# matthewdm0816/BridgeQA

Hardware: AMD Instinct MI355X
Metric: train samples/s (40k-pt scene + 512^2 view, bs16) (higher is better)
Workload: dtype bf16

## Files before the change

bridgeqa_amd/_ext.py:

```python
import ctypes
import os

import torch

from . import _cabi, gemm_route
from .gemm_route import GEMM_TILE_ROWS, TILE256_MIN_K, pick_tile

_LIB_PATH = os.environ.get("BQHIP_LIB") or os.path.join(os.path.dirname(os.path.abspath(__file__)), "lib", "libbqhip.so")

if not os.path.exists(_LIB_PATH):
    raise ImportError(
        "bridgeqa_amd: %s is missing -- build it with `python -m bridgeqa_amd.build` "
        "(hipcc --offload-arch=gfx950). There is no CPU fallback." % _LIB_PATH)

_lib = ctypes.CDLL(_LIB_PATH)
_D = _cabi.DEFINES
_cabi.bind(_lib, ("bq_abi_version", "bq_last_error"))
ABI_VERSION = _D["BQHIP_ABI_VERSION"]
if _lib.bq_abi_version() != ABI_VERSION:
    raise ImportError("bridgeqa_amd: libbqhip.so ABI %d != %d (stale library: python -m bridgeqa_amd.build --force)"
                      % (_lib.bq_abi_version(), ABI_VERSION))
_cabi.bind(_lib)
_cabi.bind(_lib, _cabi.ADDITIVE_PROTOS)
_cabi.bind(_lib, _cabi.EXTENSION_PROTOS)
# ... 1120 lines not shown
            raise RuntimeError("%s must be a contiguous float32 tensor" % n)
    W, H = int(image_dims[0]), int(image_dims[1])
    F, N = depth.shape[0], points.shape[0]
    if depth.numel() != F * W * H or frames.shape != (F, 40) or points.shape[1] != 3:
        raise RuntimeError("project_points: shapes %s %s %s" % (tuple(points.shape), tuple(depth.shape), tuple(frames.shape)))
    with torch.cuda.device(points.device):
        pix = torch.empty(F, N, dtype=torch.int32, device=points.device)
        _check(_lib.bq_project_points(_p(points), _p(depth), _p(frames), _p(pix), F, N, W, H, float(fx), float(fy), float(cx),
                                      float(cy), float(depth_min), float(depth_max), float(accuracy), _stream()),
               "project_points")
    return pix


def fuse_point_features(pix, feat, maxpool):
    if not (pix.is_cuda and feat.is_cuda):
        raise RuntimeError("fuse_point_features: CPU not supported")
    if pix.dtype != torch.int32 or feat.dtype != torch.float32 or not pix.is_contiguous() or not feat.is_contiguous():
        raise RuntimeError("fuse_point_features: pix must be contiguous int32, feat contiguous float32")
    F, N = pix.shape
    if feat.dim() != 3 or feat.shape[0] != F:
        raise RuntimeError("fuse_point_features: feat must be (F, H*W, C)")
    HW, C = feat.shape[1], feat.shape[2]
    with torch.cuda.device(pix.device):
        out = torch.empty(N, C, dtype=torch.float32, device=pix.device)
        _check(_lib.bq_fuse_point_features(_p(pix), _p(feat), _p(out), F, N, HW, C, int(bool(maxpool)), _stream()),
               "fuse_point_features")
    return out


GEMM_P_XC, GEMM_Q_XC, GEMM_OUT_F32, GEMM_BACKGROUND = (_D["BQ_GEMM_" + n] for n in ("P_XC", "Q_XC", "OUT_F32", "BACKGROUND"))
EPI_NONE, EPI_BIAS, EPI_BIAS_GELU, EPI_DGELU, EPI_BIAS_CE, EPI_ADD = (
    _D["BQ_GEMM_EPI_" + n] for n in ("NONE", "BIAS", "BIAS_GELU", "DGELU", "BIAS_CE", "ADD"))
GEMM_DET = _D["BQ_GEMM_DET"]
_GemmDesc = _cabi.STRUCTS["bq_gemm_desc"]


def _mat(t, name):
    if not t.is_cuda:
        raise RuntimeError("%s: CPU not supported (bridgeqa_amd has no CPU path)" % name)
    if t.dim() != 2 or t.stride(1) != 1:
        raise RuntimeError("%s must be a 2-D tensor with a contiguous last dimension" % name)
    return t


def _mat_rows(t, name):
    if not t.is_cuda:
        raise RuntimeError("%s: CPU not supported (bridgeqa_amd has no CPU path)" % name)
    if t.dim() == 2:
        if t.stride(1) != 1:
            raise RuntimeError("%s must have a contiguous last dimension" % name)
        return (t.shape[0], t.shape[1]), t.stride(0), 0, 0
    if t.dim() != 3 or t.stride(2) != 1:
        raise RuntimeError("%s must be (rows, cols) or a (batch, rows, cols) view with a contiguous last dimension" % name)
    B, R, C = t.shape
    ld, bs = t.stride(1), t.stride(0)
    if B == 1 or bs == R * ld:
        return (B * R, C), ld, 0, 0
    if bs < R * ld or bs % 8 or R > 65535:
        raise RuntimeError("%s: unsupported batched-row view (stride %s, shape %s)" % (name, t.stride(), tuple(t.shape)))
    return (B * R, C), ld, R, bs


def gemm_grouped(problems, flags, epilogue=EPI_NONE, tile=None, fixed_order=False):
    if _det() or fixed_order:
        return _gemm_grouped_det(problems, flags, epilogue, tile)
    return _gemm_grouped_launch(problems, flags, epilogue, tile)
# ... 6 lines not shown
    oshape, ldo, o_rpb, o_bs = _mat_rows(out, "out")
    if P.dtype != torch.bfloat16 or Q.dtype != torch.bfloat16:
        raise RuntimeError("gemm: operands must be bf16")
    if out.dtype != (torch.float32 if f32 else torch.bfloat16):
        raise RuntimeError("gemm: out must be %s" % ("float32" if f32 else "bfloat16"))
    Ni, Kc = (P.shape[1], P.shape[0]) if pxc else (P.shape[0], P.shape[1])
    Nj, Kq = (qshape[1], qshape[0]) if qxc else (qshape[0], qshape[1])
    Ni = int(pr.get("Ni", Ni))
    if (Kq != Kc and "Kc" not in pr) or tuple(oshape) != (Nj, Ni):
        raise RuntimeError("gemm: shape mismatch P%s Q%s out%s" % (tuple(P.shape), tuple(Q.shape), tuple(out.shape)))
    d.P, d.Q, d.out = P.data_ptr(), Q.data_ptr(), out.data_ptr()
    bias, out2, aux, colsum = pr.get("bias"), pr.get("out2"), pr.get("aux"), pr.get("colsum")
    if bias is not None and (bias.dtype not in (torch.float32, torch.bfloat16) or bias.numel() != Ni
                             or not bias.is_contiguous()):
        raise RuntimeError("gemm: bias must be a contiguous fp32 or bf16 (Ni,) tensor")
    d.bias_bf16 = int(bias is not None and bias.dtype == torch.bfloat16)
    n_cs = Nj if (pxc and qxc and f32) else Ni
    if epilogue != EPI_BIAS_CE and colsum is not None and (colsum.dtype != torch.float32 or colsum.numel() != n_cs
                                                           or not colsum.is_contiguous()):
        raise RuntimeError("gemm: colsum must be a contiguous fp32 (%d,) tensor" % n_cs)
    for t, nm in ((out2, "out2"), (aux, "aux")):
        if epilogue != EPI_BIAS_CE and t is not None and (t.dtype != torch.bfloat16 or t.shape != out.shape
                                                          or t.stride() != out.stride()):
            raise RuntimeError("gemm: %s must be bf16 and laid out like out" % nm)
    d.bias, d.out2, d.aux, d.colsum = _p(bias), _p(out2), _p(aux), _p(colsum)
    d.ldp, d.ldq, d.ldo = P.stride(0), ldq, ldo
    d.q_rpb, d.q_bstride, d.o_rpb, d.o_bstride = q_rpb, q_bs, o_rpb, o_bs
    d.accum = int(bool(pr.get("accum", False)))
    d.Ni, d.Nj, d.Kc = Ni, Nj, int(pr.get("Kc", Kc))
    d.p_bytes, d.q_bytes, d.ksplit = int(pr.get("p_bytes", 0)), int(pr.get("q_bytes", 0)), int(pr.get("ksplit", 1))
    return gemm_route.Shape(Ni, Nj, d.Kc, colsum is not None, bool(q_rpb or o_rpb))


def _gemm_grouped_launch(problems, flags, epilogue, tile):
    n = len(problems)
    arr = (_GemmDesc * n)()
    shapes = [_gemm_pack(arr[k], pr, flags, epilogue) for k, pr in enumerate(problems)]
    tile = int(tile or gemm_route.auto_tile(shapes, flags, epilogue))
    dev = problems[0]["out"].device
    if tile != 128:
        flags &= ~GEMM_BACKGROUND
    with torch.cuda.device(dev):
        if tile == 128 and n == 1 and (STREAMK[0] or STREAMK256[0]):
            _streamk_workspace(dev)
        _check(_lib.bq_gemm_bf16(arr, n, int(flags), int(epilogue), tile, _stream()), "gemm_bf16")


def _gemm_grouped_det(problems, flags, epilogue, tile):
    if _det() and (STREAMK[0] or STREAMK256[0]):
        raise RuntimeError("gemm: stream-K is on (streamk_enable / streamk256_enable) while the deterministic mode is on")
    f32 = bool(flags & GEMM_OUT_F32)
    probs, folds, sums = [], [], []
    for pr in problems:
        ks = int(pr.get("ksplit", 1))
        if epilogue != EPI_BIAS_CE and ks > 1:
            out = pr["out"]
            if not f32 or pr.get("colsum") is not None or pr.get("accum") or out.dim() != 2 or out.stride(1) != 1:
                raise RuntimeError("gemm: a cut contraction in the deterministic mode needs fp32 plain-row out, no colsum or accum")
            slab = torch.empty(ks, out.shape[0], out.stride(0), dtype=torch.float32, device=out.device)
            folds.append((slab, out, ks))
            pr = dict(pr, out=slab[0, :, :out.shape[1]])
        elif not f32 and epilogue != EPI_BIAS_CE and pr.get("colsum") is not None:
            sums.append((pr["out"], pr["colsum"]))
            pr = dict(pr, colsum=None)
        probs.append(pr)
    _gemm_grouped_launch(probs, flags | GEMM_DET, epilogue, tile)
    for slab, out, ks in folds:
        R, C = out.shape
        with torch.cuda.device(out.device):
            _check(_det_entry("gemm_splitk_fold")(_p(slab), _p(out), None, ks, R, C, out.stride(0), _stream()),
# ... 499 lines not shown
```

bridgeqa_amd/csrc/gemm.hip:

```cpp
#include "gemm_common.h"

namespace bq {

typedef unsigned u32x4_sk __attribute__((ext_vector_type(4)));

template <bool P_XC, bool Q_XC, int EPI, bool OUT_F32, bool SK = false>
__global__ __launch_bounds__(512) void gemm256_kernel(const GemmArgs args) {
  static_assert(!SK || (!P_XC && !Q_XC && !OUT_F32 && (EPI == EPI_NONE || EPI == EPI_BIAS)), "stream-K: K-contiguous operands, bf16 out");
  __shared__ __attribute__((aligned(16))) unsigned char smem[131072];
  __shared__ unsigned s_skflag;
  constexpr bool GTAB = !OUT_F32 && (EPI == EPI_BIAS_GELU || EPI == EPI_DGELU);
  __shared__ float s_gtab[GTAB ? GELU_TAB_N : 1];
  const int tid = threadIdx.x;
  const int lane = tid & 63;
  const int wave = __builtin_amdgcn_readfirstlane(tid >> 6);
  const int wr = wave >> 2, wc = wave & 3;

  const int nwg = args.total_tiles;
  auto xcd_order = [](int b, int n) {
    const int q = n >> 3, r = n & 7, x = b & 7;
    return (x < r ? x * (q + 1) : r * (q + 1) + (x - r) * q) + (b >> 3);
  };
  const int G = (int)gridDim.x;
  const int nkt_full = SK ? (args.p[0].Kc + 63) >> 6 : 1;
  const int U = SK ? nwg * nkt_full : 0;
  auto bound = [&](int x) {
    int b = (int)((long)x * U / G);
    const int r = b % nkt_full;
    return r == 1 ? b - 1 : (r == nkt_full - 1 ? b + 1 : b);
  };
  const int slot = SK ? xcd_order((int)blockIdx.x, G) : 0;
  int su = SK ? bound(slot) : 0;
  const int sue = SK ? bound(slot + 1) : 0;
  if (SK && su >= sue) return;
  for (;;) {
  int t, kb = 0, kseg = 0;
  if (SK) {
    t = su / nkt_full;
    kb = su - t * nkt_full;
    kseg = min(nkt_full - kb, sue - su);
  } else {
    t = xcd_order((int)blockIdx.x, nwg);
  }
  int pi = 0;
  for (int k = 1; k < args.n; ++k)
    if (t >= args.p[k].tile0) pi = k;
  const GemmProblem &pr = args.p[pi];
  const int tl = t - pr.tile0;
  const int tiles_j = (pr.Nj + 255) >> 8;
  const int bj = tiles_j - 1 - tl / pr.tiles_i(), bi = tl % pr.tiles_i();
  const int i0 = bi * 256, j0 = bj * 256;
  const int Ni = pr.Ni, Nj = pr.Nj, Kc = pr.Kc;
  const int ldp = pr.ldp, ldq = pr.ldq;
  const int nkt = SK ? kseg : (Kc + 63) >> 6;

  const auto rsP = __builtin_amdgcn_make_buffer_rsrc((void *)pr.P, 0, pr.p_bytes, 0x00020000);
  const auto rsQ = __builtin_amdgcn_make_buffer_rsrc((void *)pr.Q, 0, pr.q_bytes, 0x00020000);
  const int ur = wave * 8 + (lane >> 3);
  const int cp = lane & 7;
  unsigned voff[8];
#pragma unroll
  for (int u = 0; u < 4; ++u) {
    const int g = u & 1, half = u >> 1;
    if (!P_XC) {
      const int c = cp ^ (ur & 7);
      voff[u] = (unsigned)(((i0 + g * 128 + half * 64 + ur) * ldp + c * 8) * 2);
    } else {
      const int c = cp ^ (xg(ur) << 1);
      voff[u] = (unsigned)((ur * ldp + i0 + g * 128 + half * 64 + c * 8) * 2);
    }
  }
#pragma unroll
  for (int u = 0; u < 4; ++u) {
    const int h = u & 1, half = u >> 1;
    if (!Q_XC) {
      const int c = cp ^ (ur & 7);
      voff[4 + u] = (unsigned)(((j0 + h * 128 + (ur >> 5) * 64 + half * 32 + (ur & 31)) * ldq + c * 8) * 2);
    } else {
      const int c = cp ^ (xg(ur) << 1);
      voff[4 + u] = (unsigned)((ur * ldq + j0 + h * 128 + (c >> 2) * 64 + half * 32 + (c & 3) * 8) * 2);
    }
  }
  const unsigned p_step = P_XC ? (unsigned)(64 * ldp * 2) : 128u;
  const unsigned q_step = Q_XC ? (unsigned)(64 * ldq * 2) : 128u;
  if (SK) {
#pragma unroll
    for (int u = 0; u < 4; ++u) { voff[u] += (unsigned)kb * p_step; voff[4 + u] += (unsigned)kb * q_step; }
  }
  const unsigned lds_w = (unsigned)(wave * 1024);
  const int q_rpb = Q_XC ? (int)pr.q_rpb() : 0;
  const unsigned q_gap = (unsigned)((pr.q_bstride - q_rpb * ldq) * 2);
  int q_rl[2] = {ur, ur};

  auto stage_pair = [&](int u, int kt) {
    const bool live = kt < nkt;
    const unsigned base = (unsigned)((kt & 1) * 65536 + u * 8192) + lds_w;
#pragma unroll
    for (int d = 0; d < 2; ++d) {
      const unsigned vo = live ? voff[u + d] : 0x80000000u;
      __builtin_amdgcn_raw_ptr_buffer_load_lds(u < 4 ? rsP : rsQ, (lds_void_t *)(smem + base + d * 8192), 16, vo, 0, 0, 0);
      voff[u + d] += (u < 4) ? p_step : q_step;
    }
    if (Q_XC && u >= 4 && q_rpb != 0) {
      int &rl = q_rl[(u - 4) >> 1];
      rl += 64;
      const bool wrap = rl >= q_rpb;
      rl -= wrap ? q_rpb : 0;
      voff[u] += wrap ? q_gap : 0u;
      voff[u + 1] += wrap ? q_gap : 0u;
    }
  };

  const int row16 = lane & 15, q4 = lane >> 4;
  const int kc_base = row16 * 128 + ((q4 ^ (row16 & 7)) << 4);
  int xc_base[4];
  {
    const int q = (lane & 15) >> 2, p = lane & 3, g = (q >> 1) | ((q4 & 1) << 1);
#pragma unroll
    for (int s = 0; s < 4; ++s) xc_base[s] = (8 * q4 + q) * 128 + ((s ^ g) << 5) + 8 * p;
  }
  const int uA0 = wr * 8192, uA1 = (2 + wr) * 8192, uB0 = (4 + (wc >> 1)) * 8192, uB1 = (6 + (wc >> 1)) * 8192;
  const int bsub = (wc & 1) * 2;

  const int iw = i0 + wr * 128, jw = j0 + wc * 64;
  const bool vA0 = iw < Ni, vA1 = iw + 64 < Ni, vB0 = jw < Nj, vB1 = jw + 32 < Nj;

  f32x4 acc[8][4];
#pragma unroll
  for (int a = 0; a < 8; ++a)
#pragma unroll
    for (int b = 0; b < 4; ++b) acc[a][b] = f32x4{0.f, 0.f, 0.f, 0.f};

  constexpr bool QSUM = P_XC && Q_XC && OUT_F32;
  const bool do_qsum = QSUM && pr.colsum != nullptr && bi == 0 && wr == 0;
  f32x4 qs[4];
  bf16x8 ones;
#pragma unroll
  for (int b = 0; b < 4; ++b) qs[b] = f32x4{0.f, 0.f, 0.f, 0.f};
#pragma unroll
  for (int e = 0; e < 8; ++e) ones[e] = (__bf16)1.0f;
#define BQ_MFMA_QSUM(FB, BO)                                                                          \
  if (QSUM && do_qsum) {                                                                              \
    _Pragma("unroll") for (int kk = 0; kk < 2; ++kk) _Pragma("unroll") for (int b = 0; b < 2; ++b)    \
        qs[BO + b] = __builtin_amdgcn_mfma_f32_16x16x32_bf16(ones, FB[b][kk], qs[BO + b], 0, 0, 0);   \
  }

  stage_pair(0, 0); stage_pair(4, 0); stage_pair(6, 0); stage_pair(2, 0); stage_pair(0, 1); stage_pair(4, 1); stage_pair(6, 1);
  if (GTAB) gelu_tab_fill<EPI == EPI_DGELU>(s_gtab, tid, 512);
  asm volatile("s_waitcnt vmcnt(8)" ::: "memory");
  BQ_BARRIER();
  if (wr == 1) BQ_BARRIER();

  bf16x8 fa[4][2], fb0[2][2], fb1[2][2];
  const unsigned smem_lds = lds_addr_of(smem);
#define BQ_MFMA_Q(AO, FB, BO)                                                                         \
  _Pragma("unroll") for (int kk = 0; kk < 2; ++kk) _Pragma("unroll") for (int a = 0; a < 4; ++a)      \
      _Pragma("unroll") for (int b = 0; b < 2; ++b) acc[AO + a][BO + b] =                             \
          __builtin_amdgcn_mfma_f32_16x16x32_bf16(fa[a][kk], FB[b][kk], acc[AO + a][BO + b], 0, 0, 0);
#define BQ_PHASE_SYNC_A()                                   \
  asm volatile("s_waitcnt vmcnt(8)" ::: "memory");          \
  asm volatile("s_waitcnt lgkmcnt(0)" ::: "memory");        \
  BQ_BARRIER();                                             \
  __builtin_amdgcn_sched_barrier(0);                        \
  __builtin_amdgcn_s_setprio(1);
#define BQ_PHASE_SYNC_B()                                   \
  __builtin_amdgcn_s_setprio(0);                            \
  BQ_BARRIER();

  for (int kt = 0; kt < nkt; ++kt) {
    const unsigned buf = smem_lds + (unsigned)((kt & 1) * 65536);
    if (vA0) {
#pragma unroll
      for (int a = 0; a < 4; ++a)
#pragma unroll
        for (int kk = 0; kk < 2; ++kk) fa[a][kk] = read_frag_asm<P_XC>(buf + uA0, a, kk, kc_base, xc_base);
    }
    if (vB0) {
#pragma unroll
      for (int b = 0; b < 2; ++b)
#pragma unroll
        for (int kk = 0; kk < 2; ++kk) fb0[b][kk] = read_frag_asm<Q_XC>(buf + uB0, bsub + b, kk, kc_base, xc_base);
    }
    if (vB1) {
#pragma unroll
      for (int b = 0; b < 2; ++b)
#pragma unroll
        for (int kk = 0; kk < 2; ++kk) fb1[b][kk] = read_frag_asm<Q_XC>(buf + uB1, bsub + b, kk, kc_base, xc_base);
    }
    stage_pair(2, kt + 1);
    BQ_PHASE_SYNC_A();
    if (vA0 && vB0) { BQ_MFMA_Q(0, fb0, 0) }
    if (vB0) { BQ_MFMA_QSUM(fb0, 0) }
    if (vA0 && vB1) { BQ_MFMA_Q(0, fb1, 2) }
    if (vB1) { BQ_MFMA_QSUM(fb1, 2) }
    BQ_PHASE_SYNC_B();
    if (vA1) {
#pragma unroll
      for (int a = 0; a < 4; ++a)
#pragma unroll
        for (int kk = 0; kk < 2; ++kk) fa[a][kk] = read_frag_asm<P_XC>(buf + uA1, a, kk, kc_base, xc_base);
    }
    stage_pair(0, kt + 2); stage_pair(4, kt + 2); stage_pair(6, kt + 2);
    BQ_PHASE_SYNC_A();
// ... 927 lines not shown
  for (int k = 0; k < ga.n; ++k) long_k = long_k && ga.p[k].Kc >= 64 * long_k_tiles;
  int rc = -1;
  with_gemm_form(pxc, qxc, f32, epi, [&](auto PX, auto QX, auto F32, auto E) {
    constexpr bool P = decltype(PX)::value, Q = decltype(QX)::value, F = decltype(F32)::value;
    constexpr int EP = decltype(E)::value;
    rc = det ? launch_variant<P, Q, EP, F, FORM_DET>(ga, tile, st, false) : launch_variant<P, Q, EP, F>(ga, tile, st, long_k);
  });
  return rc;
}

}

extern "C" int bq_gemm_max_problems(void) { return bq::GEMM_MAX_PROBLEMS; }

extern "C" int bq_gemm_bf16(const bq_gemm_desc *d, int n, int flags, int epilogue, int tile, void *stream) {
  using namespace bq;
  BQ_REQUIRE(epilogue >= BQ_GEMM_EPI_NONE && epilogue <= BQ_GEMM_EPI_ADD, BQ_EINVAL, "bq_gemm_bf16: unknown epilogue %d", epilogue);
  BQ_REQUIRE(d != nullptr && n >= 1, BQ_EINVAL, "bq_gemm_bf16: no problems");
  BQ_REQUIRE(tile == 256 || tile == 128 || tile == 64 || tile == 32, BQ_EINVAL,
             "bq_gemm_bf16: tile must be 256, 128 (= 256 x 128), 64 or 32 (got %d)", tile);
  const bool pxc = flags & BQ_GEMM_P_XC, qxc = flags & BQ_GEMM_Q_XC, f32 = flags & BQ_GEMM_OUT_F32;
  BQ_REQUIRE(!(flags & BQ_GEMM_BACKGROUND) || tile == 128, BQ_EINVAL, "bq_gemm_bf16: BQ_GEMM_BACKGROUND needs tile 128");
  const bool det = flags & BQ_GEMM_DET;
  BQ_REQUIRE(!det || tile != 128 || gemm_sk_mode() == 0, BQ_EINVAL,
             "bq_gemm_bf16: BQ_GEMM_DET with a stream-K mode on (bq_gemm_streamk_mode)");
  hipStream_t st = (hipStream_t)stream;
  int done = 0;
  while (done < n) {
    GemmArgs ga;
    ga.n = 0;
    ga.total_tiles = 0;
    while (done < n && ga.n < GEMM_MAX_PROBLEMS) {
      const bq_gemm_desc &s = d[done];
      BQ_REQUIRE(s.P && s.Q && s.out, BQ_EINVAL, "bq_gemm_bf16: null operand (problem %d)", done);
      BQ_REQUIRE(s.Ni > 0 && s.Nj > 0 && s.Kc > 0, BQ_EINVAL, "bq_gemm_bf16: empty problem %d", done);
      BQ_REQUIRE(s.ldp % 8 == 0 && s.ldq % 8 == 0, BQ_EINVAL, "bq_gemm_bf16: operand leading dimensions must be multiples of 8 elements");
      BQ_REQUIRE(s.Ni % 8 == 0 && s.ldo % (f32 ? 4 : 8) == 0, BQ_EINVAL, "bq_gemm_bf16: Ni and ldo must be multiples of 8 (Ni = %d, ldo = %d)", s.Ni, s.ldo);
      BQ_REQUIRE(!qxc || s.Nj % 8 == 0, BQ_EINVAL, "bq_gemm_bf16: a contraction-major Q needs Nj %% 8 == 0 (Nj = %d)", s.Nj);
      BQ_REQUIRE((pxc && qxc) || s.Kc % 64 == 0, BQ_EINVAL,
                 "bq_gemm_bf16: a K-contiguous operand needs Kc %% 64 == 0 (Kc = %d; zero-pad the other operand and pass "
                 "p_bytes / q_bytes when the rows are shorter)", s.Kc);
      BQ_REQUIRE(((uintptr_t)s.P % 16 == 0) && ((uintptr_t)s.Q % 16 == 0) && ((uintptr_t)s.out % 16 == 0), BQ_EINVAL,
                 "bq_gemm_bf16: operands must be 16-byte aligned");
      BQ_REQUIRE(epilogue != EPI_BIAS_GELU || s.out2, BQ_EINVAL, "bq_gemm_bf16: BIAS_GELU needs out2");
      BQ_REQUIRE(epilogue != EPI_DGELU || s.aux, BQ_EINVAL, "bq_gemm_bf16: DGELU needs aux");
      BQ_REQUIRE(epilogue != EPI_ADD || s.aux, BQ_EINVAL, "bq_gemm_bf16: ADD needs aux");
      BQ_REQUIRE((epilogue != EPI_ADD && epilogue != EPI_DGELU && tile != 128) || ((long)s.Nj + 256) * s.ldo * (f32 ? 4 : 2) < 0x7FFFFFFFL,
                 BQ_EINVAL, "bq_gemm_bf16: out / aux larger than 2 GB (problem %d)", done);
      const long pb = pxc ? ((long)(s.Kc - 1) * s.ldp + s.Ni) * 2 : ((long)(s.Ni - 1) * s.ldp + s.Kc) * 2;
      long qb = qxc ? ((long)(s.Kc - 1) * s.ldq + s.Nj) * 2 : ((long)(s.Nj - 1) * s.ldq + s.Kc) * 2;
      const int tj = tile == 256 ? 256 : tile, ti = (tile == 256 || tile == 128) ? 256 : 64;
      BQ_REQUIRE(s.q_rpb >= 0 && s.o_rpb >= 0 && s.q_rpb <= 65535 && s.o_rpb <= 65535, BQ_EINVAL,
                 "bq_gemm_bf16: q_rpb / o_rpb must be in 0..65535 (problem %d)", done);
      long q_span = 0, o_span = 0;
      if (s.q_rpb > 0) {
        const long rows = qxc ? s.Kc : s.Nj, cols = qxc ? s.Nj : s.Kc;
        BQ_REQUIRE(rows % s.q_rpb == 0 && s.q_bstride % 8 == 0 && (long)s.q_bstride >= (long)s.q_rpb * s.ldq, BQ_EINVAL,
                   "bq_gemm_bf16: q map: rows %ld must be whole batches of q_rpb = %d rows, q_bstride %% 8 == 0 and >= q_rpb * ldq",
                   rows, s.q_rpb);
        BQ_REQUIRE(tile != 256 || (qxc && s.q_rpb >= 64), BQ_EINVAL,
                   "bq_gemm_bf16: tile 256 maps only the contraction rows of a contraction-major Q, q_rpb >= 64");
        BQ_REQUIRE(tile != 128 || !qxc, BQ_EINVAL, "bq_gemm_bf16: tile 128 has no map on a contraction-major Q");
        q_span = (rows / s.q_rpb - 1) * (long)s.q_bstride + (long)(s.q_rpb - 1) * s.ldq + cols;
        qb = q_span * 2;
      }
      if (s.o_rpb > 0) {
// ... 9 lines not shown
      BQ_REQUIRE(pb + (long)ti * s.ldp * 2 < 0x7FFFFFFFL && qb + (long)tj * s.ldq * 2 + (s.q_rpb > 0 ? 2L * s.q_bstride * 2 : 0) < 0x7FFFFFFFL,
                 BQ_EINVAL, "bq_gemm_bf16: operand larger than 2 GB (problem %d)", done);
      BQ_REQUIRE(!det || f32 || epilogue == EPI_BIAS_CE || !s.colsum, BQ_EINVAL,
                 "bq_gemm_bf16: BQ_GEMM_DET: column sums of a bf16 output are float atomics (use bq_colsum_grouped_det_bf16)");
      BQ_REQUIRE(!det || epilogue == EPI_BIAS_CE || s.ksplit <= 1 || (!s.colsum && !s.accum && s.o_rpb == 0), BQ_EINVAL,
                 "bq_gemm_bf16: BQ_GEMM_DET: a cut contraction takes no colsum, accum or output map (problem %d)", done);
      GemmProblem &g = ga.p[ga.n];
      g.P = (const __bf16 *)s.P; g.Q = (const __bf16 *)s.Q; g.out = s.out; g.bias = s.bias; g.out2 = s.out2;
      g.aux = (const __bf16 *)s.aux; g.colsum = s.colsum;
      g.ldp = s.ldp; g.ldq = s.ldq; g.ldo = s.ldo; g.Ni = s.Ni; g.Nj = s.Nj; g.Kc = s.Kc;
      g.flags = (s.bias_bf16 != 0 ? 1 : 0) | (s.accum != 0 ? 2 : 0);
      g.rpb_pack = (int)((unsigned)s.q_rpb | ((unsigned)s.o_rpb << 16));
      g.q_bstride = s.q_bstride; g.o_bstride = s.o_bstride;
      g.p_bytes = (unsigned)(s.p_bytes > 0 ? s.p_bytes : pb);
      g.q_bytes = (unsigned)((s.q_bytes > 0 && s.q_rpb == 0) ? s.q_bytes : qb);
      int ks_ = 1;
      if (epilogue == EPI_BIAS_CE) {
        BQ_REQUIRE(s.out2 && s.aux && s.colsum && s.ksplit > 0 && s.ksplit <= s.Ni && s.ksplit <= 65535 && tile == 256, BQ_EINVAL,
                   "bq_gemm_bf16: the cross-entropy epilogue needs out2 (partials), aux (targets), colsum (target logits), "
                   "ksplit = valid vocabulary entries (<= 65535), tile 256");
        ks_ = s.ksplit;
      } else {
        BQ_REQUIRE(s.ksplit <= 1 || (f32 && tile != 256), BQ_EINVAL, "bq_gemm_bf16: ksplit needs fp32 out and tile 64");
        BQ_REQUIRE(s.ksplit <= 65535, BQ_ELIMIT, "bq_gemm_bf16: ksplit = %d > 65535", s.ksplit);
        BQ_REQUIRE(s.ksplit <= 1 || epilogue == EPI_NONE, BQ_EINVAL, "bq_gemm_bf16: ksplit needs the NONE epilogue");
        ks_ = (f32 && tile != 256 && s.ksplit > 1) ? s.ksplit : 1;
      }
      BQ_REQUIRE((s.Ni + ti - 1) / ti <= 65535, BQ_ELIMIT, "bq_gemm_bf16: Ni = %d too wide", s.Ni);
      g.tiles_ks = (int)((unsigned)((s.Ni + ti - 1) / ti) | ((unsigned)ks_ << 16));
      g.tile0 = ga.total_tiles;
      ga.total_tiles += g.tiles_i() * ((s.Nj + tj - 1) / tj) * (epilogue == EPI_BIAS_CE ? 1 : g.ksplit());
      ++ga.n;
      ++done;
    }
    BQ_REQUIRE(launch_gemm(ga, flags, epilogue, tile, st) == 0, BQ_EINVAL,
               "bq_gemm_bf16: unsupported combination flags=%d epilogue=%d tile=%d", flags, epilogue, tile);
    int rc = check_launch("gemm_bf16");
    if (rc) return rc;
  }
  return 0;
}

extern "C" int bq_colsum_grouped_bf16(const bq_colsum_desc *d, int n, void *stream) {
  using namespace bq;
  BQ_REQUIRE(d != nullptr && n >= 1, BQ_EINVAL, "bq_colsum_grouped_bf16: no problems");
  hipStream_t st = (hipStream_t)stream;
  int done = 0;
  while (done < n) {
    ColsumArgs ca;
    ca.n = 0;
    int wgs = 0;
    while (done < n && ca.n < COLSUM_MAX_PROBLEMS) {
      const bq_colsum_desc &s = d[done];
      BQ_REQUIRE(s.g && s.out && s.M > 0 && s.N > 0, BQ_EINVAL, "bq_colsum_grouped_bf16: bad problem %d", done);
      BQ_REQUIRE(s.N % 8 == 0 && s.ld % 8 == 0 && ((uintptr_t)s.g % 16 == 0), BQ_EINVAL,
                 "bq_colsum_grouped_bf16: N and ld must be multiples of 8, g 16-byte aligned");
      ColsumProblem &c = ca.p[ca.n];
      c.g = (const __bf16 *)s.g; c.out = s.out; c.M = s.M; c.N = s.N; c.ld = s.ld;
      c.cblocks = (s.N + 255) / 256;
      c.wg0 = wgs;
      wgs += c.cblocks * ((s.M + COLSUM_ROWS - 1) / COLSUM_ROWS);
      ++ca.n;
      ++done;
    }
    hipLaunchKernelGGL(colsum_grouped_kernel, dim3(wgs), dim3(256), 0, st, ca);
    int rc = check_launch("colsum_grouped");
// ... 375 lines not shown
```

bridgeqa_amd/csrc/gemm_common.h:

```cpp
#pragma once
#include <type_traits>

#include "bq_common.h"

namespace bq {

typedef __bf16 bf16x8 __attribute__((ext_vector_type(8)));
typedef __bf16 bf16x4 __attribute__((ext_vector_type(4)));
typedef float f32x4 __attribute__((ext_vector_type(4)));
typedef __attribute__((address_space(3))) bf16x4 lds_bf16x4_t;
typedef __attribute__((address_space(3))) void lds_void_t;

enum { EPI_NONE = 0, EPI_BIAS = 1, EPI_BIAS_GELU = 2, EPI_DGELU = 3, EPI_BIAS_CE = 4, EPI_ADD = 5 };

struct GemmProblem {
  const __bf16 *P, *Q;
  void *out;
  const void *bias;
  void *out2;
  const __bf16 *aux;
  float *colsum;
  int ldp, ldq, ldo;
  int Ni, Nj, Kc;
  int tile0;
  unsigned p_bytes, q_bytes;
  int q_bstride, o_bstride;
  int rpb_pack;
  int tiles_ks;
  int flags;
  __host__ __device__ __forceinline__ int q_rpb() const { return rpb_pack & 0xffff; }
  __host__ __device__ __forceinline__ int o_rpb() const { return (int)((unsigned)rpb_pack >> 16); }
  __host__ __device__ __forceinline__ int tiles_i() const { return tiles_ks & 0xffff; }
  __host__ __device__ __forceinline__ int ksplit() const { return (int)((unsigned)tiles_ks >> 16); }
  __host__ __device__ __forceinline__ int bias_bf16() const { return flags & 1; }
  __host__ __device__ __forceinline__ int accum() const { return (flags >> 1) & 1; }
};
static_assert(sizeof(GemmProblem) == 112, "GemmProblem grew: GEMM_MAX_PROBLEMS x sizeof must stay below the 4 KB kernarg limit");

__device__ __forceinline__ unsigned mapped_row(int r, int ld, int rpb, int bstride) {
  if (rpb == 0) return (unsigned)(r * ld);
  const int b = r / rpb;
  return (unsigned)(b * bstride + (r - b * rpb) * ld);
}

__device__ __forceinline__ void load_bias4(const GemmProblem &pr, int i, float (&bv)[4]) {
  if (pr.bias_bf16()) {
    const bf16x4 b = *reinterpret_cast<const bf16x4 *>(reinterpret_cast<const __bf16 *>(pr.bias) + i);
    bv[0] = (float)b[0]; bv[1] = (float)b[1]; bv[2] = (float)b[2]; bv[3] = (float)b[3];
  } else {
    const float4 b = *reinterpret_cast<const float4 *>(reinterpret_cast<const float *>(pr.bias) + i);
    bv[0] = b.x; bv[1] = b.y; bv[2] = b.z; bv[3] = b.w;
  }
}

constexpr int GEMM_MAX_PROBLEMS = 36;
struct GemmArgs {
  int n;
  int total_tiles;
  GemmProblem p[GEMM_MAX_PROBLEMS];
  void *sk_ws;
};
constexpr long SK_TICKET_BYTES = 65536, SK_SLAB_BYTES = 256 * 128 * 4;
// ... 189 lines not shown
```

bridgeqa_amd/fusion_wgrad.py:

```python
import os

import torch
import torch.nn.functional as F

from .fusion_state import *
from .fusion_state import __all__ as _state_all
from .gemm_route import DW_TILE as _DW_TILE, SHORT_DW_MIN_ROWS as _SHORT_DW_MIN_ROWS
from .gemm_route import SHORT_DW_TILE as _SHORT_DW_TILE, wgrad_class

_NATIVE_GEMM = [True]


def _rows(t):
    t2 = t.reshape(-1, t.shape[-1])
    if t2.dtype != torch.bfloat16:
        t2 = t2.to(torch.bfloat16)
    if t2.stride(1) != 1 or t2.stride(0) % 8 or t2.data_ptr() % 16:
        t2 = t2.contiguous()
    return t2


def _native_ok(t, N, K):
    return _NATIVE_GEMM[0] and t.is_cuda and compute_dtype() == torch.bfloat16 and K % 64 == 0 and N % 8 == 0

# ... 32 lines not shown
            db = g2.sum(0, dtype=torch.float32)
    return dw, db


_DEFER = [None]


def begin_deferred_wgrad():
    _DEFER[0] = []


def _accumulate_grad(p, g):
    if p is None or not p.requires_grad:
        return
    if p.grad is None:
        p.grad = g
    else:
        p.grad.add_(g)


def take_deferred_wgrad():
    items, _DEFER[0] = _DEFER[0], None
    return items or []


def flush_deferred_wgrad():
    flush_deferred_items(take_deferred_wgrad())


_PLAN_CACHE = {}
_PLAN_WGRAD = [True]
_QSUM = [True]
_QSUM64 = [True]


def plan_big_launches(tiles, cus, max_problems=36, moved_cost=0.011):
    key = (tuple(tiles), cus, max_problems)
    hit = _PLAN_CACHE.get(key)
    if hit is not None:
        return hit
    n = len(tiles)
    rounds = lambda t: -(-t // cus) if t > 0 else 0
    order = sorted(range(n), key=lambda k: tiles[k])
    default = [list(range(n))[i:i + max_problems] for i in range(0, n, max_problems)]
    best = (sum(rounds(sum(tiles[k] for k in g)) for g in default), default, [])
    if n <= 2 * max_problems:
        for m in range(0, min(6, n)):
            moved = order[:m]
            rest = order[m:]
            cost_moved = moved_cost * sum(tiles[k] for k in moved)
            by_size = {}
            for k in rest:
                by_size.setdefault(tiles[k], []).append(k)
            sizes = sorted(by_size)
            if len(sizes) > 5:
                break
            total, cnt = sum(tiles[k] for k in rest), len(rest)
            combos = [[]]
            for sz in sizes:
                combos = [c + [x] for c in combos for x in range(len(by_size[sz]) + 1)]
                if len(combos) > 50000:
                    combos = None
                    break
            if combos is None:
                break
            for c in combos:
                nb = sum(c)
                if nb > max_problems or cnt - nb > max_problems:
                    continue
                tb = sum(x * sz for x, sz in zip(c, sizes))
                cost = rounds(tb) + rounds(total - tb) + cost_moved
                if cost < best[0] - 1e-9:
                    gb = [k for x, sz in zip(c, sizes) for k in by_size[sz][:x]]
                    ga = [k for x, sz in zip(c, sizes) for k in by_size[sz][x:]]
                    best = (cost, [g for g in (ga, gb) if g], list(moved))
    plan = (best[1], best[2])
    _PLAN_CACHE[key] = plan
    return plan


def _nrows(t):
    return t.shape[0] if t.dim() == 2 else t.shape[0] * t.shape[1]


def flush_deferred_items(items):
    if not items:
        return
    from . import _ext
    flags = _ext.GEMM_P_XC | _ext.GEMM_Q_XC | _ext.GEMM_OUT_F32
    items = [tuple(it) + (None,) * (5 - len(it)) for it in items]
    dws = [None] * len(items)
    prim = [k for k, it in enumerate(items) if it[4] is None]
    second = [k for k, it in enumerate(items) if it[4] is not None]
    cls = {k: wgrad_class(_nrows(items[k][0]), (items[k][0].shape[-1], items[k][1].shape[-1], items[k][0].dim() == 2))
           for k in prim}
    big, mid, small = ([k for k in prim if cls[k] == c] for c in ("big", "mid", "small"))
    if _PLAN_WGRAD[0]:
        big.sort(key=lambda k: -_nrows(items[k][0]))
    groups = [big] if big else []
    if big and _PLAN_WGRAD[0]:
        tj = _DW_TILE[0]
        tiles = [-(-items[k][0].shape[-1] // tj) * -(-items[k][1].shape[-1] // 256) for k in big]
        cus = torch.cuda.get_device_properties(items[big[0]][0].device).multi_processor_count
        plan_groups, moved = plan_big_launches(tiles, cus * (256 // tj))
        groups = [[big[j] for j in g] for g in plan_groups]
        small = small + [big[j] for j in moved]
    dbs = {}
    for tile, idx_groups in ((_DW_TILE[0], groups), (_SHORT_DW_TILE[0], [mid] if mid else []), (64, [small] if small else [])):
        for idx in idx_groups:
            probs = []
            for k in idx:
                g2, x2 = items[k][0], items[k][1]
                dws[k] = torch.empty(g2.shape[-1], x2.shape[-1], dtype=torch.float32, device=g2.device)
                pr = dict(P=x2, Q=g2, out=dws[k])
                if items[k][3] is not None and _QSUM[0] and (tile != 64 or _QSUM64[0]):
                    dbs[k] = torch.empty(g2.shape[-1], dtype=torch.float32, device=g2.device)
                    pr["colsum"] = dbs[k]
                probs.append(pr)
            _ext.gemm_grouped(probs, flags, _ext.EPI_NONE, tile)
    with_b = [k for k in prim if items[k][3] is not None and k not in dbs]
    if with_b:
        dbs.update(zip(with_b, _ext.colsum_grouped([items[k][0].reshape(-1, items[k][0].shape[-1]) for k in with_b])))
    if second:
        probs = []
        for k in second:
            g2, x2, pk = items[k][0], items[k][1], items[k][4]
            pr = dict(P=x2, Q=g2, out=dws[pk], accum=True)
            if items[pk][3] is not None:
                pr["colsum"] = dbs[pk]
            probs.append(pr)
        _ext.gemm_grouped(probs, flags, _ext.EPI_NONE, 64)
    for k in prim:
        g2, x2, ws, bs = items[k][:4]
        n = g2.shape[-1] // len(ws)
        for j, w in enumerate(ws):
            _accumulate_grad(w, dws[k][j * n:(j + 1) * n] if len(ws) > 1 else dws[k].view(w.shape))
            if bs is not None:
                _accumulate_grad(bs[j], dbs[k][j * n:(j + 1) * n] if len(ws) > 1 else dbs[k])


def _defer_ok(g2, x2):
    return (_DEFER[0] is not None and _NATIVE_GEMM[0] and g2.is_cuda and g2.dtype == torch.bfloat16
            and x2.dtype == torch.bfloat16 and g2.shape[1] % 8 == 0 and x2.shape[1] % 8 == 0)


def _park(g2, x2, ws, bs):
    _DEFER[0].append((_rows(g2), _rows(x2), ws, bs))
# ... 11 lines not shown
```

include/bqhip_fusion.h:

```cpp
#ifndef BQHIP_FUSION_H
#define BQHIP_FUSION_H
#include "bqhip.h"
#include "bqhip_lstm.h"
#include "bqhip_scene.h"
#include "bqhip_view.h"
#include "bqhip_beam.h"

#ifdef __cplusplus
extern "C" {
#endif

BQ_API int bq_attn_fwd(const void *Q, const void *K, const void *V, void *O, float *LSE, const float *mask, int B,
                       int H, int Lq, int Lk, int Lkp, long q_bs, long q_rs, long q_hs, long k_bs, long k_rs,
                       long k_hs, long o_bs, long o_rs, long o_hs, float scale, float p_drop, unsigned seed,
                       const unsigned *seed_ptr, int causal, void *stream);

BQ_API int bq_attn_bwd(const void *Q, const void *K, const void *V, const void *dO, const float *LSE, const void *O,
                       float *DELTA, const float *mask, void *dQ, void *dK, void *dV, int B, int H, int Lq, int Lk,
                       int Lkp, long q_bs, long q_rs, long q_hs, long k_bs, long k_rs, long k_hs, long g_bs, long g_rs,
                       long g_hs, float scale, float p_drop, unsigned seed, const unsigned *seed_ptr, int causal,
                       void *stream);

typedef struct bq_attn_side {
  const void *Q, *K, *V, *dO, *O;
// ... 124 lines not shown
                                   const void *dy, const float *mean, const float *rstd, void *dx, void *dresidual,
                                   float *dgb, int M, int H, float eps, float p_drop, unsigned seed,
                                   const unsigned *seed_ptr, void *stream);

BQ_API int bq_adamw_chunk_elems(void);
BQ_API int bq_adamw_tensor_bytes(void);
BQ_API int bq_adamw_multi(const void *table, const void *chunks, int n_chunks, const float *step, float beta1,
                          float beta2, float eps, float grad_clip_value, void *stream);

BQ_API int bq_box_point_count(const float *points, const float *center, const float *size, const float *heading, int *count,
                              int B, int N, int ld, int K, int cap, void *stream);
BQ_API int bq_nms(const float *box, const float *score, const int *cls, const unsigned char *valid, unsigned char *keep,
                  int B, int K, float thresh, int old_type, int same_cls, void *stream);
BQ_API int bq_nms_f64(const float *box, const float *score, const int *cls, const unsigned char *valid, unsigned char *keep,
                      int B, int K, double thresh, int old_type, int same_cls, void *stream);

BQ_API int bq_ap_match(const double *box_tab, const int *det_box, const double *gt_tab, const int *seg_det,
                       const int *seg_gt, const double *thresholds, unsigned char *tp, double *ovmax, int *jmax, int Nb,
                       int D, int G, int S, int T, int max_seg_gt, void *stream);
BQ_API int bq_ap_curve(const unsigned char *tp, const int *cls_off, const double *npos, double *rec, double *prec,
                       double *ap, double *last_recall, int D, int C, int T, void *stream);

BQ_API int bq_project_points(const float *points, const float *depth, const float *frames, int *pix, int F, int N, int W,
                             int H, float fx, float fy, float cx, float cy, float depth_min, float depth_max,
                             float accuracy, void *stream);
BQ_API int bq_fuse_point_features(const int *pix, const float *feat, float *out, int F, int N, int HW, int C, int maxpool,
                                  void *stream);

#define BQ_GEMM_P_XC 1
#define BQ_GEMM_Q_XC 2
#define BQ_GEMM_OUT_F32 4
#define BQ_GEMM_BACKGROUND 8
#define BQ_GEMM_DET 16
#define BQ_GEMM_EPI_NONE 0
#define BQ_GEMM_EPI_BIAS 1
#define BQ_GEMM_EPI_BIAS_GELU 2
#define BQ_GEMM_EPI_DGELU 3
#define BQ_GEMM_EPI_ADD 5
#define BQ_GEMM_EPI_BIAS_CE 4
typedef struct bq_gemm_desc {
  const void *P, *Q;
  void *out;
  const float *bias;
  void *out2;
  const void *aux;
  float *colsum;
  int ldp, ldq, ldo;
  int Ni, Nj, Kc;
  int bias_bf16;
  long p_bytes, q_bytes;
  int ksplit;
  int q_rpb, q_bstride, o_rpb, o_bstride;
  int accum;
} bq_gemm_desc;
BQ_API int bq_gemm_max_problems(void);
BQ_API int bq_gemm_bf16(const bq_gemm_desc *problems, int n, int flags, int epilogue, int tile, void *stream);
BQ_API long bq_gemm_workspace_bytes(void);
BQ_API int bq_gemm_set_workspace(void *ws, long bytes, void *stream);
BQ_API int bq_gemm_streamk_mode(int mode);

typedef struct bq_colsum_desc {
  const void *g;
  float *out;
  int M, N, ld;
} bq_colsum_desc;
BQ_API int bq_colsum_grouped_bf16(const bq_colsum_desc *problems, int n, void *stream);
// ... 98 lines not shown
```

Baseline: 493.1.

## Fold second row source into weight-gradient GEMM K loop on tile 256

Weight-gradient problems that share a weight (two input/grad pairs) now run as one 256-tile GEMM whose K loop continues from the first operand pair into the second, switching buffer resources and offsets mid-loop. This replaces a separate launch or problem for the second contribution plus its accumulation, so each output tile is written once. It adds a descriptor flag, host validation, table-splitting logic for the problem limit, and per-iteration branch overhead in the kernel's staging path.

```diff
diff --git a/bridgeqa_amd/_ext.py b/bridgeqa_amd/_ext.py
--- a/bridgeqa_amd/_ext.py
+++ b/bridgeqa_amd/_ext.py
@@ -1176,6 +1176,7 @@
 EPI_NONE, EPI_BIAS, EPI_BIAS_GELU, EPI_DGELU, EPI_BIAS_CE, EPI_ADD = (
     _D["BQ_GEMM_EPI_" + n] for n in ("NONE", "BIAS", "BIAS_GELU", "DGELU", "BIAS_CE", "ADD"))
 GEMM_DET = _D["BQ_GEMM_DET"]
+GEMM_SECOND = _D["BQ_GEMM_SECOND"]
 _GemmDesc = _cabi.STRUCTS["bq_gemm_desc"]
 
 
@@ -1248,10 +1249,34 @@
     return gemm_route.Shape(Ni, Nj, d.Kc, colsum is not None, bool(q_rpb or o_rpb))
 
 
+def _gemm_pack_second(d, pr, prim):
+    if pr.get("P2") is None or pr.get("Q2") is None:
+        raise RuntimeError("gemm: a second row source needs both P2 and Q2")
+    P2, Q2 = _mat(pr["P2"], "P2"), pr["Q2"]
+    qshape, ldq, q_rpb, q_bs = _mat_rows(Q2, "Q2")
+    if P2.dtype != torch.bfloat16 or Q2.dtype != torch.bfloat16:
+        raise RuntimeError("gemm: operands must be bf16")
+    if P2.shape[0] != qshape[0] or P2.shape[1] != prim.Ni or qshape[1] != prim.Nj:
+        raise RuntimeError("gemm: shape mismatch P2%s Q2%s for a (%d, %d) weight gradient" % (
+            tuple(P2.shape), tuple(Q2.shape), prim.Nj, prim.Ni))
+    d.P, d.Q = P2.data_ptr(), Q2.data_ptr()
+    d.ldp, d.ldq, d.q_rpb, d.q_bstride = P2.stride(0), ldq, q_rpb, q_bs
+    d.Ni, d.Nj, d.Kc, d.ksplit = prim.Ni, prim.Nj, P2.shape[0], 1
+
+
 def _gemm_grouped_launch(problems, flags, epilogue, tile):
-    n = len(problems)
+    two = [("P2" in pr) or ("Q2" in pr) for pr in problems]
+    n = len(problems) + sum(two)
     arr = (_GemmDesc * n)()
-    shapes = [_gemm_pack(arr[k], pr, flags, epilogue) for k, pr in enumerate(problems)]
+    shapes, k = [], 0
+    for pr, second in zip(problems, two):
+        shapes.append(_gemm_pack(arr[k], pr, flags, epilogue))
+        k += 1
+        if second:
+            _gemm_pack_second(arr[k], pr, arr[k - 1])
+            k += 1
+    if any(two):
+        flags |= GEMM_SECOND
     tile = int(tile or gemm_route.auto_tile(shapes, flags, epilogue))
     dev = problems[0]["out"].device
     if tile != 128:
diff --git a/bridgeqa_amd/csrc/gemm.hip b/bridgeqa_amd/csrc/gemm.hip
--- a/bridgeqa_amd/csrc/gemm.hip
+++ b/bridgeqa_amd/csrc/gemm.hip
@@ -52,10 +52,21 @@
   const int i0 = bi * 256, j0 = bj * 256;
   const int Ni = pr.Ni, Nj = pr.Nj, Kc = pr.Kc;
   const int ldp = pr.ldp, ldq = pr.ldq;
-  const int nkt = SK ? kseg : (Kc + 63) >> 6;
+  constexpr bool SEG = P_XC && Q_XC && OUT_F32 && !SK;
+  bool has_b = false;
+  if constexpr (SEG) has_b = pr.has_seg() != 0;
+  const GemmProblem &sg = args.p[SEG && has_b ? pi + 1 : pi];
+  int nkt_a = 0, nkt_b = 0;
+  if constexpr (SEG) {
+    nkt_a = (Kc + 63) >> 6;
+    nkt_b = has_b ? (sg.Kc + 63) >> 6 : 0;
+  }
+  const int nkt = SK ? kseg : ((Kc + 63) >> 6) + nkt_b;
 
   const auto rsP = __builtin_amdgcn_make_buffer_rsrc((void *)pr.P, 0, pr.p_bytes, 0x00020000);
   const auto rsQ = __builtin_amdgcn_make_buffer_rsrc((void *)pr.Q, 0, pr.q_bytes, 0x00020000);
+  const auto rsPb = SEG ? __builtin_amdgcn_make_buffer_rsrc((void *)sg.P, 0, sg.p_bytes, 0x00020000) : rsP;
+  const auto rsQb = SEG ? __builtin_amdgcn_make_buffer_rsrc((void *)sg.Q, 0, sg.q_bytes, 0x00020000) : rsQ;
   const int ur = wave * 8 + (lane >> 3);
   const int cp = lane & 7;
   unsigned voff[8];
@@ -88,9 +99,11 @@
     for (int u = 0; u < 4; ++u) { voff[u] += (unsigned)kb * p_step; voff[4 + u] += (unsigned)kb * q_step; }
   }
   const unsigned lds_w = (unsigned)(wave * 1024);
-  const int q_rpb = Q_XC ? (int)pr.q_rpb() : 0;
+  int q_rpb = Q_XC ? (int)pr.q_rpb() : 0;
   const unsigned q_gap = (unsigned)((pr.q_bstride - q_rpb * ldq) * 2);
   int q_rl[2] = {ur, ur};
+  auto rsP0 = rsP, rsP2 = rsP, rsQc = rsQ;
+  unsigned p_step0 = p_step, p_step2 = p_step;
 
   auto stage_pair = [&](int u, int kt) {
     const bool live = kt < nkt;
@@ -98,8 +111,13 @@
 #pragma unroll
     for (int d = 0; d < 2; ++d) {
       const unsigned vo = live ? voff[u + d] : 0x80000000u;
-      __builtin_amdgcn_raw_ptr_buffer_load_lds(u < 4 ? rsP : rsQ, (lds_void_t *)(smem + base + d * 8192), 16, vo, 0, 0, 0);
-      voff[u + d] += (u < 4) ? p_step : q_step;
+      if constexpr (SEG) {
+        __builtin_amdgcn_raw_ptr_buffer_load_lds(u < 4 ? (u < 2 ? rsP0 : rsP2) : rsQc, (lds_void_t *)(smem + base + d * 8192), 16, vo, 0, 0, 0);
+        voff[u + d] += (u < 4) ? (u < 2 ? p_step0 : p_step2) : q_step;
+      } else {
+        __builtin_amdgcn_raw_ptr_buffer_load_lds(u < 4 ? rsP : rsQ, (lds_void_t *)(smem + base + d * 8192), 16, vo, 0, 0, 0);
+        voff[u + d] += (u < 4) ? p_step : q_step;
+      }
     }
     if (Q_XC && u >= 4 && q_rpb != 0) {
       int &rl = q_rl[(u - 4) >> 1];
@@ -110,6 +128,25 @@
       voff[u + 1] += wrap ? q_gap : 0u;
     }
   };
+  auto roll = [&](int k1, int k2) {
+    const int c = cp ^ (xg(ur) << 1);
+    const unsigned pcol = (unsigned)(ur * sg.ldp + i0 + c * 8), step_b = (unsigned)(64 * sg.ldp * 2);
+    if (k1 == nkt_a) {
+      voff[2] = (pcol + 64u) * 2u; voff[3] = (pcol + 192u) * 2u;
+      rsP2 = rsPb; p_step2 = step_b;
+    }
+    if (k2 == nkt_a) {
+      voff[0] = pcol * 2u; voff[1] = (pcol + 128u) * 2u;
+      rsP0 = rsPb; p_step0 = step_b;
+      rsQc = rsQb; q_rpb = 0;
+    }
+    if (k2 >= nkt_a) {
+      const unsigned qcol = mapped_row((k2 - nkt_a) * 64 + ur, sg.ldq, sg.q_rpb(), sg.q_bstride) +
+                            (unsigned)(j0 + (c >> 2) * 64 + (c & 3) * 8);
+#pragma unroll
+      for (int u = 0; u < 4; ++u) voff[4 + u] = (qcol + (unsigned)((u & 1) * 128 + (u >> 1) * 32)) * 2u;
+    }
+  };
 
   const int row16 = lane & 15, q4 = lane >> 4;
   const int kc_base = row16 * 128 + ((q4 ^ (row16 & 7)) << 4);
@@ -145,7 +182,11 @@
         qs[BO + b] = __builtin_amdgcn_mfma_f32_16x16x32_bf16(ones, FB[b][kk], qs[BO + b], 0, 0, 0);   \
   }
 
-  stage_pair(0, 0); stage_pair(4, 0); stage_pair(6, 0); stage_pair(2, 0); stage_pair(0, 1); stage_pair(4, 1); stage_pair(6, 1);
+  stage_pair(0, 0); stage_pair(4, 0); stage_pair(6, 0); stage_pair(2, 0);
+  if constexpr (SEG) {
+    if (has_b && 1 >= nkt_a) roll(-1, 1);
+  }
+  stage_pair(0, 1); stage_pair(4, 1); stage_pair(6, 1);
   if (GTAB) gelu_tab_fill<EPI == EPI_DGELU>(s_gtab, tid, 512);
   asm volatile("s_waitcnt vmcnt(8)" ::: "memory");
   BQ_BARRIER();
@@ -169,6 +210,9 @@
 
   for (int kt = 0; kt < nkt; ++kt) {
     const unsigned buf = smem_lds + (unsigned)((kt & 1) * 65536);
+    if constexpr (SEG) {
+      if (has_b && kt + 2 >= nkt_a) roll(kt + 1, kt + 2);
+    }
     if (vA0) {
 #pragma unroll
       for (int a = 0; a < 4; ++a)
@@ -1162,6 +1206,10 @@
     ga.total_tiles = 0;
     while (done < n && ga.n < GEMM_MAX_PROBLEMS) {
       const bq_gemm_desc &s = d[done];
+      const bool has2 = (flags & BQ_GEMM_SECOND) && done + 1 < n && d[done + 1].out == nullptr;
+      if (has2 && ga.n + 2 > GEMM_MAX_PROBLEMS) break;
+      BQ_REQUIRE(s.out || !(flags & BQ_GEMM_SECOND), BQ_EINVAL,
+                 "bq_gemm_bf16: BQ_GEMM_SECOND: entry %d has no out and no primary problem in front of it", done);
       BQ_REQUIRE(s.P && s.Q && s.out, BQ_EINVAL, "bq_gemm_bf16: null operand (problem %d)", done);
       BQ_REQUIRE(s.Ni > 0 && s.Nj > 0 && s.Kc > 0, BQ_EINVAL, "bq_gemm_bf16: empty problem %d", done);
       BQ_REQUIRE(s.ldp % 8 == 0 && s.ldq % 8 == 0, BQ_EINVAL, "bq_gemm_bf16: operand leading dimensions must be multiples of 8 elements");
@@ -1237,6 +1285,44 @@
       ga.total_tiles += g.tiles_i() * ((s.Nj + tj - 1) / tj) * (epilogue == EPI_BIAS_CE ? 1 : g.ksplit());
       ++ga.n;
       ++done;
+      if (has2) {
+        const bq_gemm_desc &t = d[done];
+        BQ_REQUIRE(tile == 256 && pxc && qxc && f32 && epilogue == EPI_NONE, BQ_EINVAL,
+                   "bq_gemm_bf16: a second row source needs the weight-gradient form (P_XC | Q_XC | OUT_F32, epilogue NONE) on "
+                   "tile 256 (entry %d)", done);
+        BQ_REQUIRE(t.P && t.Q && ((uintptr_t)t.P % 16 == 0) && ((uintptr_t)t.Q % 16 == 0) && t.ldp % 8 == 0 && t.ldq % 8 == 0,
+                   BQ_EINVAL, "bq_gemm_bf16: second row source: null / unaligned operand or leading dimension (entry %d)", done);
+        BQ_REQUIRE(t.Ni == s.Ni && t.Nj == s.Nj && t.Kc > 0, BQ_EINVAL,
+                   "bq_gemm_bf16: second row source: Ni / Nj must equal the primary's (%d x %d against %d x %d), Kc > 0 (entry %d)",
+                   t.Ni, t.Nj, s.Ni, s.Nj, done);
+        BQ_REQUIRE(s.ksplit <= 1 && t.ksplit <= 1 && !t.accum && !t.bias && !t.out2 && !t.aux && !t.colsum && t.o_rpb == 0, BQ_EINVAL,
+                   "bq_gemm_bf16: second row source: no ksplit, and nothing but P, Q, their leading dimensions, Kc and the q map "
+                   "(entry %d)", done);
+        BQ_REQUIRE(t.q_rpb >= 0 && t.q_rpb <= 65535, BQ_EINVAL, "bq_gemm_bf16: second row source: q_rpb must be in 0..65535 (entry %d)", done);
+        const long pb2 = ((long)(t.Kc - 1) * t.ldp + t.Ni) * 2;
+        long qb2 = ((long)(t.Kc - 1) * t.ldq + t.Nj) * 2, q_reach = ((long)(t.Kc + 64) * t.ldq + t.Nj + 256) * 2;
+        if (t.q_rpb > 0) {
+          BQ_REQUIRE(t.Kc % t.q_rpb == 0 && t.q_bstride % 8 == 0 && (long)t.q_bstride >= (long)t.q_rpb * t.ldq, BQ_EINVAL,
+                     "bq_gemm_bf16: second row source: q map: Kc = %d must be whole batches of q_rpb = %d rows, q_bstride %% 8 == 0 "
+                     "and >= q_rpb * ldq", t.Kc, t.q_rpb);
+          qb2 = ((t.Kc / t.q_rpb - 1) * (long)t.q_bstride + (long)(t.q_rpb - 1) * t.ldq + t.Nj) * 2;
+          q_reach = (((long)(t.Kc + 63) / t.q_rpb + 1) * t.q_bstride + (long)t.q_rpb * t.ldq + t.Nj + 256) * 2;
+        }
+        BQ_REQUIRE(pb2 + 256L * t.ldp * 2 < 0x7FFFFFFFL && q_reach < 0x7FFFFFFFL, BQ_EINVAL,
+                   "bq_gemm_bf16: second row source: operand larger than 2 GB (entry %d)", done);
+        g.flags |= 4;
+        GemmProblem &c = ga.p[ga.n];
+        c = GemmProblem{};
+        c.P = (const __bf16 *)t.P; c.Q = (const __bf16 *)t.Q;
+        c.ldp = t.ldp; c.ldq = t.ldq; c.Ni = t.Ni; c.Nj = t.Nj; c.Kc = t.Kc;
+        c.p_bytes = (unsigned)pb2; c.q_bytes = (unsigned)qb2;
+        c.q_bstride = t.q_bstride;
+        c.rpb_pack = t.q_rpb;
+        c.flags = 8;
+        c.tile0 = 0x7fffffff;
+        ++ga.n;
+        ++done;
+      }
     }
     BQ_REQUIRE(launch_gemm(ga, flags, epilogue, tile, st) == 0, BQ_EINVAL,
                "bq_gemm_bf16: unsupported combination flags=%d epilogue=%d tile=%d", flags, epilogue, tile);
diff --git a/bridgeqa_amd/csrc/gemm_common.h b/bridgeqa_amd/csrc/gemm_common.h
--- a/bridgeqa_amd/csrc/gemm_common.h
+++ b/bridgeqa_amd/csrc/gemm_common.h
@@ -28,6 +28,7 @@
   int rpb_pack;
   int tiles_ks;
   int flags;
+  __host__ __device__ __forceinline__ int has_seg() const { return (flags >> 2) & 1; }
   __host__ __device__ __forceinline__ int q_rpb() const { return rpb_pack & 0xffff; }
   __host__ __device__ __forceinline__ int o_rpb() const { return (int)((unsigned)rpb_pack >> 16); }
   __host__ __device__ __forceinline__ int tiles_i() const { return tiles_ks & 0xffff; }
diff --git a/bridgeqa_amd/fusion_wgrad.py b/bridgeqa_amd/fusion_wgrad.py
--- a/bridgeqa_amd/fusion_wgrad.py
+++ b/bridgeqa_amd/fusion_wgrad.py
@@ -88,6 +88,7 @@
 _PLAN_WGRAD = [True]
 _QSUM = [True]
 _QSUM64 = [True]
+_TWO_SOURCE = [True]
 
 
 def plan_big_launches(tiles, cus, max_problems=36, moved_cost=0.011):
@@ -135,6 +136,25 @@
     return plan
 
 
+def split_for_table(group, two, max_entries=36):
+    entries = len(group) + sum(two)
+    n = -(-entries // max_entries)
+    if n <= 1:
+        return [list(group)]
+    chunks = [group[c::n] for c in range(n)]
+    sizes = [len(group[c::n]) + sum(two[c::n]) for c in range(n)]
+    if max(sizes) > max_entries:
+        chunks, cur, used = [], [], 0
+        for k, t in zip(group, two):
+            if used + 1 + t > max_entries:
+                chunks.append(cur)
+                cur, used = [], 0
+            cur.append(k)
+            used += 1 + t
+        chunks.append(cur)
+    return [c for c in chunks if c]
+
+
 def _nrows(t):
     return t.shape[0] if t.dim() == 2 else t.shape[0] * t.shape[1]
 
@@ -161,6 +181,14 @@
         plan_groups, moved = plan_big_launches(tiles, cus * (256 // tj))
         groups = [[big[j] for j in g] for g in plan_groups]
         small = small + [big[j] for j in moved]
+    attach = {}
+    if _TWO_SOURCE[0] and _DW_TILE[0] == 256:
+        on_big = {k for g in groups for k in g}
+        for k in second:
+            if items[k][4] in on_big and (items[k][3] is None or _QSUM[0]):
+                attach.setdefault(items[k][4], k)
+        second = [k for k in second if attach.get(items[k][4]) != k]
+        groups = [c for g in groups for c in split_for_table(g, [k in attach for k in g])]
     dbs = {}
     for tile, idx_groups in ((_DW_TILE[0], groups), (_SHORT_DW_TILE[0], [mid] if mid else []), (64, [small] if small else [])):
         for idx in idx_groups:
@@ -169,6 +197,8 @@
                 g2, x2 = items[k][0], items[k][1]
                 dws[k] = torch.empty(g2.shape[-1], x2.shape[-1], dtype=torch.float32, device=g2.device)
                 pr = dict(P=x2, Q=g2, out=dws[k])
+                if k in attach:
+                    pr.update(P2=items[attach[k]][1], Q2=items[attach[k]][0])
                 if items[k][3] is not None and _QSUM[0] and (tile != 64 or _QSUM64[0]):
                     dbs[k] = torch.empty(g2.shape[-1], dtype=torch.float32, device=g2.device)
                     pr["colsum"] = dbs[k]
diff --git a/include/bqhip_fusion.h b/include/bqhip_fusion.h
--- a/include/bqhip_fusion.h
+++ b/include/bqhip_fusion.h
@@ -180,6 +180,7 @@
 #define BQ_GEMM_OUT_F32 4
 #define BQ_GEMM_BACKGROUND 8
 #define BQ_GEMM_DET 16
+#define BQ_GEMM_SECOND 32
 #define BQ_GEMM_EPI_NONE 0
 #define BQ_GEMM_EPI_BIAS 1
 #define BQ_GEMM_EPI_BIAS_GELU 2
```

New measurement: 499.6 (median of 6 runs). 1.01x the previous value.
